# retir/Style-Big-GAN

Hardware: AMD Instinct MI355X
Metric: images/sec (G+D step) StyleGAN2-ADA 256x256 bf16 (higher is better)
Workload: dtype bf16; 1 GPU; configs/sg2ada.yaml @ 256x256: sg2_classic G (skip) + D (orig), softplus + R1(0.01)/4, idle Greg slot /16 (G lr x 16/17), global batch 64 = 1 rank(s) x 2 round(s) x batch_gpu 32 (the rounds of a phase evaluated in one pass, minibatch-std groups and loss those of the separate rounds), bf16 from 8x8 up (num_fp16_res 6; the reference recipe defaults to 4), conv_clamp 256, ADA off; global_batch=64, per_rank_batch=64, parallelism=dp1

## Files before the change

### include/sbg_hip.h

```cpp
#ifndef SBG_HIP_H
#define SBG_HIP_H

#include <stdint.h>

#ifdef __cplusplus
extern "C" {
#endif

typedef void* sbg_stream_t;

enum sbg_status {
    SBG_OK = 0,
    SBG_ERR_INVALID = 1,
    SBG_ERR_UNSUPPORTED = 2,
    SBG_ERR_LAUNCH = 3
};

enum sbg_dtype { SBG_F32 = 0, SBG_F16 = 1, SBG_BF16 = 2 };

enum sbg_act {
    SBG_ACT_LINEAR = 1, SBG_ACT_RELU = 2, SBG_ACT_LRELU = 3, SBG_ACT_TANH = 4, SBG_ACT_SIGMOID = 5,
    SBG_ACT_ELU = 6, SBG_ACT_SELU = 7, SBG_ACT_SOFTPLUS = 8, SBG_ACT_SWISH = 9
};

// ... 14 lines not shown
    float gain;
    int     inSize[4];      int64_t inStride[4];
    int     filterSize[2];  int     filterStride[2];
    int     outSize[4];     int64_t outStride[4];
    const float* oscale; const float* noise; int64_t noise_stride_n; const float* bias;
    int act; float alpha, act_gain, clamp;
    int     filter_exact16;
    const void* dact_y; float* dact_partial; int dact_act; float dact_alpha, dact_gain, dact_clamp;
    const float* post_scale;
} sbg_upfirdn2d_params;
int sbg_upfirdn2d_tail_supported(const sbg_upfirdn2d_params* p);
int64_t sbg_upfirdn2d_dact_rows(const sbg_upfirdn2d_params* p);
int sbg_upfirdn2d(const sbg_upfirdn2d_params* p, sbg_stream_t stream);

int sbg_upfirdn2d_separable_supported(int up, int down, int taps);
int sbg_upfirdn2d_separable(const float* x, const float* f, float* y, int M, int IH, int IW, int OH, int OW, int taps,
                            int up, int down, int padx0, int pady0, int flip, float gain, sbg_stream_t stream);

#define SBG_MAX_TAPS 16
typedef struct sbg_conv_params {
    const void* x; const void* w; void* y;
    const float* oscale;
    int xdtype, ydtype;
    int N, IH, IW, Cin, Cout, OH, OW;
    int64_t xs_n, xs_h, xs_w;
    int64_t ys_n, ys_h, ys_w;
    int64_t ws_slab, ws_co;
    int stride;
    int ntaps;
    int tap_dy[SBG_MAX_TAPS], tap_dx[SBG_MAX_TAPS], tap_slab[SBG_MAX_TAPS];
    int accumulate;
    const float* bias; const float* noise; int64_t noise_stride_n;
    int act; float alpha, gain, clamp;
    void* workspace; int ksplit;
    int nphase; int ph_ntaps[4], ph_oh[4], ph_ow[4]; int64_t ph_yoff[4];
} sbg_conv_params;
int64_t sbg_conv2d_igemm_workspace(const sbg_conv_params* p);
int     sbg_conv2d_igemm(const sbg_conv_params* p, sbg_stream_t stream);


typedef struct sbg_wgrad_params {
    const void* a; const void* b; float* out; void* workspace;
    int dtype;
    int N, PH, PW, Ca, BH, BW, Cb;
    int64_t as_n, as_h, as_w;
    int64_t bs_n, bs_h, bs_w;
    int stride;
    int ntaps;
    int tap_dy[SBG_MAX_TAPS], tap_dx[SBG_MAX_TAPS];
    int accumulate;
} sbg_wgrad_params;
int64_t sbg_conv2d_wgrad_workspace(const sbg_wgrad_params* p);
int     sbg_conv2d_wgrad(const sbg_wgrad_params* p, sbg_stream_t stream);


int sbg_scale_nc(const void* x, const float* a, const float* z, void* y, int dtype, int layout,
                 int N, int C, int64_t HW, int64_t z_stride_n, sbg_stream_t stream);
int sbg_scale_shift_nc(const void* x, const float* a, const float* b, void* y, int dtype, int layout,
                       int N, int C, int64_t HW, sbg_stream_t stream);

int sbg_dot_hw_splits(int layout, int N, int C, int64_t HW);
int sbg_dot_hw(const void* u, const void* v, float* partial, int dtype, int layout,
               int N, int C, int64_t HW, sbg_stream_t stream);
int sbg_moments_hw(const void* x, float* r, int dtype, int N, int C, int64_t HW, sbg_stream_t stream);

typedef struct sbg_gg_problem {
    const float *a0, *b0, *a1, *b1;
    float* c; const float* bias; float* rowsum;
    int64_t a0_rs, a0_cs, b0_rs, b0_cs, a1_rs, a1_cs, b1_rs, b1_cs, c_rs, c_cs;
    int M, N, K0, K1, nterms;
    float alpha0, alpha1, bias_scale, rowsum_scale;
} sbg_gg_problem;
int sbg_grouped_gemm(const sbg_gg_problem* problems, int count, sbg_stream_t stream);

int sbg_dot_hw_scale_supported(int C);
int sbg_dot_hw_scale(const void* u, const void* v, const float* scale, void* y, float* partial, int dtype,
                     int N, int C, int64_t HW, sbg_stream_t stream);


int sbg_modconv_bwd_supported(int C);
int sbg_modconv_bwd(const void* dy, const void* y, const float* dcoef, const float* noise, const float* bias,
                    void* d2, float* partial, float* dnoise, int dtype, int N, int C, int64_t HW, int64_t noise_stride_n,
                    int act, float alpha, float gain, float clamp, sbg_stream_t stream);
int sbg_modconv_bwd_prescaled(const void* dy, const void* y, const float* prescale, const float* dcoef, const float* noise, const float* bias,
                              void* d2, float* partial, float* partial3, float* dnoise, int dtype, int N, int C, int64_t HW,
                              int64_t noise_stride_n, int act, float alpha, float gain, float clamp, sbg_stream_t stream);

int64_t sbg_sn_workspace(int rows, int cols);
int sbg_sn_power_iteration(const float* W, const float* u, float* v, float* u_new, float* sigma, void* workspace,
                           int rows, int cols, float eps, sbg_stream_t stream);

int64_t sbg_mbstd_workspace(int N, int C, int HW, int G, int F);
int sbg_mbstd_fwd(const float* x, float* y, void* workspace, int N, int C, int HW, int G, int F, sbg_stream_t stream);
int sbg_mbstd_bwd(const float* x, const float* dy, float* dx, int N, int C, int HW, int G, int F, sbg_stream_t stream);

int sbg_split_bf16_cat(const float* x, void* y, int64_t outer, int64_t C, int64_t inner, int nseg, const int* order, sbg_stream_t stream);
int sbg_split_bf16_cat_nd(const float* x, const int64_t* shape, const int64_t* xstrides, int cat_dim, void* y, int nseg, const int* order, sbg_stream_t stream);

int sbg_attention_supported(int Q, int M, int D, int DV);
int sbg_attention_fwd(const float* theta, const float* phi, const float* g, float* out, int N, int Q, int M, int D, int DV,
                      sbg_stream_t stream);
int sbg_attention_bwd_supported(int Q, int M, int D, int DV);
int64_t sbg_attention_bwd_workspace(int N, int Q);
int sbg_attention_bwd(const float* theta, const float* phi, const float* g, const float* dout, float* dtheta, float* dphi, float* dg,
                      void* workspace, int N, int Q, int M, int D, int DV, sbg_stream_t stream);

// ... 152 lines not shown
```

### style-big-gan_amd/_lib.py

```python
import ctypes
import os
import threading

import torch

_HERE = os.path.dirname(os.path.abspath(__file__))
LIB_PATH = os.environ.get("SBG_HIP_LIBRARY") or os.path.join(_HERE, "libsbg_hip.so")

SBG_F32, SBG_F16, SBG_BF16 = 0, 1, 2
SBG_MAX_TAPS = 16

_DTYPES = {torch.float32: SBG_F32, torch.float16: SBG_F16, torch.bfloat16: SBG_BF16}


def dtype_code(dtype):
    try:
        return _DTYPES[dtype]
    except KeyError:
        raise RuntimeError(f"style_big_gan_amd: unsupported dtype {dtype} (float32 / float16 / bfloat16 only)")


class UpfirdnParams(ctypes.Structure):
    _fields_ = [
        ("x", ctypes.c_void_p), ("f", ctypes.c_void_p), ("y", ctypes.c_void_p),
# ... 60 lines not shown
class GgProblem(ctypes.Structure):
    _fields_ = [("a0", ctypes.c_void_p), ("b0", ctypes.c_void_p), ("a1", ctypes.c_void_p), ("b1", ctypes.c_void_p),
                ("c", ctypes.c_void_p), ("bias", ctypes.c_void_p), ("rowsum", ctypes.c_void_p),
                ("a0_rs", ctypes.c_int64), ("a0_cs", ctypes.c_int64), ("b0_rs", ctypes.c_int64), ("b0_cs", ctypes.c_int64),
                ("a1_rs", ctypes.c_int64), ("a1_cs", ctypes.c_int64), ("b1_rs", ctypes.c_int64), ("b1_cs", ctypes.c_int64),
                ("c_rs", ctypes.c_int64), ("c_cs", ctypes.c_int64),
                ("M", ctypes.c_int), ("N", ctypes.c_int), ("K0", ctypes.c_int), ("K1", ctypes.c_int), ("nterms", ctypes.c_int),
                ("alpha0", ctypes.c_float), ("alpha1", ctypes.c_float), ("bias_scale", ctypes.c_float), ("rowsum_scale", ctypes.c_float)]


class ProfRecord(ctypes.Structure):
    _fields_ = [("kind", ctypes.c_int), ("dims", ctypes.c_int * 7), ("flops", ctypes.c_double), ("bytes", ctypes.c_double),
                ("ms", ctypes.c_float), ("pad", ctypes.c_int)]


KERNEL_KINDS = {1: "bias_act", 2: "upfirdn2d", 3: "conv_igemm", 4: "conv_wgrad", 5: "wgrad_reduce", 6: "scale_nc", 7: "dot_hw", 9: "sn_power", 10: "attention",
                11: "grid_sample", 12: "filter1d", 13: "color", 14: "weight_prep", 15: "torgb", 16: "fromrgb", 17: "grouped_gemm", 18: "ppl",
                19: "projector", 20: "image_export", 21: "resample", 22: "pr", 23: "grad_finish", 24: "resident", 25: "diffaug", 26: "nn_u8", 27: "swd", 28: "spectrum",
                29: "msssim"}
MSSSIM_VARIANTS = {0: "level", 1: "down", 2: "merge"}
SWD_VARIANTS = {0: "pyr_down", 1: "pyr_lap", 2: "gather", 3: "moments", 4: "project", 5: "l1", 6: "merge"}
SPECTRUM_VARIANTS = {0: "rows", 1: "cols"}
NN_VARIANTS = {0: "norms", 1: "single", 2: "split", 3: "merge"}
RESIDENT_PATHS = {1: "dword", 2: "byte"}
PPL_VARIANTS = {0: "slerp", 1: "lerp", 2: "prep", 3: "dist"}
PROJ_VARIANTS = {0: "reg", 1: "reg_bwd", 2: "normalize", 3: "sqdist", 4: "sqdist_bwd"}
IMG_VARIANTS = {0: "quantize_tile", 1: "truncate_mix"}
QUANT_RULES = {"grid": 0, "clamp": 1}
RESAMPLE_VARIANTS = {0: "h", 1: "v"}
PR_VARIANTS = {0: "single", 1: "split", 2: "merge", 3: "norms"}
GRAD_FINISH_VARIANTS = {0: "sweep", 1: "merge"}
DIFFAUG_VARIANTS = {0: "sum", 1: "apply", 2: "adj_sum", 3: "adj_apply", 4: "single", 5: "adj_single"}
DIFFAUG_WORDS = 12
ATT_VARIANTS = {0: "single", 1: "stream", 2: "stream_stats", 3: "stream_dq", 4: "stream_dkv"}

_lib = None
_lock = threading.Lock()

_c = ctypes
SYMBOLS = [
    ("sbg_version", _c.c_int, []),
    ("sbg_last_error", _c.c_char_p, []),
    ("sbg_bias_act", _c.c_int, [_c.c_void_p] * 6 + [_c.c_int, _c.c_int, _c.c_int, _c.c_float, _c.c_float, _c.c_float,
                                                   _c.c_int64, _c.c_int, _c.c_int64, _c.c_void_p]),
    ("sbg_upfirdn2d_tail_supported", _c.c_int, [_c.POINTER(UpfirdnParams)]),
    ("sbg_upfirdn2d", _c.c_int, [_c.POINTER(UpfirdnParams), _c.c_void_p]),
    ("sbg_upfirdn2d_dact_rows", _c.c_int64, [_c.POINTER(UpfirdnParams)]),
    ("sbg_upfirdn2d_separable_supported", _c.c_int, [_c.c_int] * 3),
    ("sbg_upfirdn2d_separable", _c.c_int, [_c.c_void_p] * 3 + [_c.c_int] * 11 + [_c.c_float, _c.c_void_p]),
    ("sbg_conv2d_igemm_workspace", _c.c_int64, [_c.POINTER(ConvParams)]),
    ("sbg_conv2d_igemm", _c.c_int, [_c.POINTER(ConvParams), _c.c_void_p]),
    ("sbg_conv2d_wgrad_workspace", _c.c_int64, [_c.POINTER(WgradParams)]),
    ("sbg_conv2d_wgrad", _c.c_int, [_c.POINTER(WgradParams), _c.c_void_p]),
    ("sbg_scale_nc", _c.c_int, [_c.c_void_p] * 4 + [_c.c_int, _c.c_int, _c.c_int, _c.c_int, _c.c_int64, _c.c_int64, _c.c_void_p]),
    ("sbg_scale_shift_nc", _c.c_int, [_c.c_void_p] * 4 + [_c.c_int, _c.c_int, _c.c_int, _c.c_int, _c.c_int64, _c.c_void_p]),
    ("sbg_sn_workspace", _c.c_int64, [_c.c_int, _c.c_int]),
    ("sbg_sn_power_iteration", _c.c_int, [_c.c_void_p] * 6 + [_c.c_int, _c.c_int, _c.c_float, _c.c_void_p]),
    ("sbg_mbstd_workspace", _c.c_int64, [_c.c_int] * 5),
    ("sbg_mbstd_fwd", _c.c_int, [_c.c_void_p] * 3 + [_c.c_int] * 5 + [_c.c_void_p]),
    ("sbg_mbstd_bwd", _c.c_int, [_c.c_void_p] * 3 + [_c.c_int] * 5 + [_c.c_void_p]),
    ("sbg_split_bf16_cat", _c.c_int, [_c.c_void_p, _c.c_void_p, _c.c_int64, _c.c_int64, _c.c_int64, _c.c_int, _c.POINTER(_c.c_int), _c.c_void_p]),
    ("sbg_split_bf16_cat_nd", _c.c_int, [_c.c_void_p, _c.POINTER(_c.c_int64), _c.POINTER(_c.c_int64), _c.c_int, _c.c_void_p, _c.c_int, _c.POINTER(_c.c_int), _c.c_void_p]),
    ("sbg_attention_supported", _c.c_int, [_c.c_int] * 4),
    ("sbg_attention_fwd", _c.c_int, [_c.c_void_p] * 4 + [_c.c_int] * 5 + [_c.c_void_p]),
    ("sbg_attention_bwd_supported", _c.c_int, [_c.c_int] * 4),
    ("sbg_attention_bwd_workspace", _c.c_int64, [_c.c_int, _c.c_int]),
    ("sbg_attention_bwd", _c.c_int, [_c.c_void_p] * 8 + [_c.c_int] * 5 + [_c.c_void_p]),
    ("sbg_dot_hw_splits", _c.c_int, [_c.c_int, _c.c_int, _c.c_int, _c.c_int64]),
    ("sbg_dot_hw", _c.c_int, [_c.c_void_p] * 3 + [_c.c_int, _c.c_int, _c.c_int, _c.c_int, _c.c_int64, _c.c_void_p]),
    ("sbg_moments_hw", _c.c_int, [_c.c_void_p, _c.c_void_p, _c.c_int, _c.c_int, _c.c_int, _c.c_int64, _c.c_void_p]),
    ("sbg_grouped_gemm", _c.c_int, [_c.c_void_p, _c.c_int, _c.c_void_p]),
    ("sbg_dot_hw_scale_supported", _c.c_int, [_c.c_int]),
    ("sbg_dot_hw_scale", _c.c_int, [_c.c_void_p] * 5 + [_c.c_int, _c.c_int, _c.c_int, _c.c_int64, _c.c_void_p]),
    ("sbg_modconv_bwd_supported", _c.c_int, [_c.c_int]),
    ("sbg_modconv_bwd", _c.c_int, [_c.c_void_p] * 8 + [_c.c_int, _c.c_int, _c.c_int, _c.c_int64, _c.c_int64, _c.c_int, _c.c_float, _c.c_float, _c.c_float, _c.c_void_p]),
    ("sbg_modconv_bwd_prescaled", _c.c_int, [_c.c_void_p] * 10 + [_c.c_int, _c.c_int, _c.c_int, _c.c_int64, _c.c_int64, _c.c_int, _c.c_float, _c.c_float, _c.c_float, _c.c_void_p]),
    ("sbg_pack_weight", _c.c_int, [_c.c_void_p, _c.c_void_p, _c.c_int, _c.c_int, _c.c_int, _c.c_int, _c.c_int] + [_c.c_int64] * 4
     + [_c.c_int, _c.c_float, _c.c_void_p, _c.c_void_p]),
    ("sbg_unpack_wgrad", _c.c_int, [_c.c_void_p, _c.c_int64, _c.c_int64, _c.c_void_p, _c.c_void_p, _c.c_void_p] + [_c.c_int] * 4
     + [_c.c_int64] * 4 + [_c.c_float, _c.c_void_p]),
    ("sbg_demod_coefs", _c.c_int, [_c.c_void_p] * 3 + [_c.c_int] * 3 + [_c.c_float, _c.c_void_p]),
    ("sbg_demod_coefs_bwd", _c.c_int, [_c.c_void_p] * 6 + [_c.c_int] * 3 + [_c.c_void_p]),
    ("sbg_torgb_supported", _c.c_int, [_c.c_int, _c.c_int]),
    ("sbg_torgb_bwd_blocks", _c.c_int, [_c.c_int, _c.c_int, _c.c_int64]),
    ("sbg_torgb_fwd", _c.c_int, [_c.c_void_p] * 4 + [_c.c_int] * 4 + [_c.c_int64, _c.c_float, _c.c_void_p]),
    ("sbg_torgb_bwd", _c.c_int, [_c.c_void_p] * 6 + [_c.c_int] * 4 + [_c.c_int64, _c.c_float, _c.c_void_p]),
    ("sbg_fromrgb_supported", _c.c_int, [_c.c_int] * 3),
    ("sbg_fromrgb_bwd_blocks", _c.c_int, [_c.c_int, _c.c_int64]),
    ("sbg_fromrgb_fwd", _c.c_int, [_c.c_void_p] * 4 + [_c.c_int] * 4 + [_c.c_int64, _c.c_int, _c.c_float, _c.c_float, _c.c_float, _c.c_void_p]),
    ("sbg_fromrgb_bwd", _c.c_int, [_c.c_void_p] * 6 + [_c.c_int] * 4 + [_c.c_int64, _c.c_int, _c.c_float, _c.c_float, _c.c_float, _c.c_void_p]),
    ("sbg_grid_sample2d", _c.c_int, [_c.POINTER(GridSampleParams), _c.c_void_p]),
    ("sbg_grid_sample2d_bwd", _c.c_int, [_c.POINTER(GridSampleParams), _c.c_void_p]),
    ("sbg_grid_sample2d_bwd_overwrites", _c.c_int, [_c.POINTER(GridSampleParams)]),
    ("sbg_color_transform", _c.c_int, [_c.c_void_p] * 3 + [_c.c_int, _c.c_int64, _c.c_void_p]),
    ("sbg_filter1d_batch", _c.c_int, [_c.c_void_p] * 3 + [_c.c_int] * 8 + [_c.c_void_p]),
    ("sbg_ppl_slerp_endpoints", _c.c_int, [_c.c_void_p] * 3 + [_c.c_float, _c.c_void_p, _c.c_int, _c.c_int, _c.c_void_p]),
    ("sbg_ppl_lerp_endpoints", _c.c_int, [_c.c_void_p] * 3 + [_c.c_float, _c.c_void_p, _c.c_int, _c.c_int64, _c.c_void_p]),
    ("sbg_ppl_prep_images", _c.c_int, [_c.c_void_p] * 2 + [_c.c_int] * 4 + [_c.c_int64] * 4 + [_c.c_int, _c.c_int, _c.c_void_p]),
    ("sbg_ppl_dist_workspace", _c.c_int64, [_c.c_int, _c.c_int64]),
    ("sbg_ppl_dist", _c.c_int, [_c.c_void_p] * 3 + [_c.c_int, _c.c_int64, _c.c_float, _c.c_void_p]),
    ("sbg_proj_noise_reg_workspace", _c.c_int64, [_c.c_void_p, _c.c_int]),
    ("sbg_proj_noise_reg", _c.c_int, [_c.c_void_p] * 2 + [_c.c_int] + [_c.c_void_p] * 4),
    ("sbg_proj_noise_reg_bwd", _c.c_int, [_c.c_void_p] * 3 + [_c.c_int] + [_c.c_void_p] * 4),
    ("sbg_proj_noise_normalize_workspace", _c.c_int64, [_c.c_void_p, _c.c_int]),
    ("sbg_proj_noise_normalize", _c.c_int, [_c.c_void_p] * 2 + [_c.c_int] + [_c.c_void_p] * 2),
    ("sbg_proj_sqdist_workspace", _c.c_int64, [_c.c_int64]),
# ... 113 lines not shown
```

### style-big-gan_amd/csrc/conv_wgrad.hip

```cpp
#include "conv_common.h"
#include "lds_asm.h"

namespace {

using sbgconv::bf16_mfma; using sbgconv::f16_mfma; using sbgconv::Mfma;

struct WgradArgs {
    const unsigned short* a; const unsigned short* b; float* out; float* ws;
    int N, PH, PW, Ca, BH, BW, Cb;
    int64_t as_n, as_h, as_w, bs_n, bs_h, bs_w;
    int stride, ntaps;
    int tap_dy[SBG_MAX_TAPS], tap_dx[SBG_MAX_TAPS];
    int accumulate;
    int64_t P;
    int nchunks;
    int nsplit, chunks_per_split;
    int atiles, btiles;
    int tap0;
    int ntaps_total;
};

static __device__ __forceinline__ bool wgrad_decode_block(const WgradArgs& p, int& ta, int& tb, int& split)
{
    const int T = p.atiles * p.btiles;
// ... 102 lines not shown
    };

    if (chunk_begin < chunk_end) {
        issue_loads(chunk_begin);
        for (int c = chunk_begin; c < chunk_end; c++) {
            write_tiles();
            __syncthreads();
            if (c + 1 < chunk_end) issue_loads(c + 1);
            short8_t fa[TA];
#pragma unroll
            for (int i = 0; i < TA; i++) fa[i] = read_frag(sA, RSA, wa + 16 * i);
#pragma unroll
            for (int t = 0; t < NT; t++) {
                if (t < p.ntaps) {
                    short8_t fb[TB];
#pragma unroll
                    for (int j = 0; j < TB; j++) fb[j] = read_frag(sB + t * B_BYTES, RSB, wb + 16 * j);
#pragma unroll
                    for (int i = 0; i < TA; i++)
#pragma unroll
                        for (int j = 0; j < TB; j++) acc[t][i][j] = Mfma<MF>::run(fa[i], fb[j], acc[t][i][j]);
                }
            }
            __syncthreads();
        }
    }

    const bool direct = (p.nsplit == 1);
    float* dst_base = direct ? p.out : p.ws + (int64_t)split * p.ntaps_total * p.Ca * p.Cb;
#pragma unroll
    for (int t = 0; t < NT; t++) {
        if (t >= p.ntaps) continue;
        float* slab = dst_base + (int64_t)(p.tap0 + t) * p.Ca * p.Cb;
#pragma unroll
        for (int i = 0; i < TA; i++)
#pragma unroll
            for (int j = 0; j < TB; j++) {
                const int cb = cb0 + wb + 16 * j + fi;
                if (cb >= p.Cb) continue;
#pragma unroll
                for (int e = 0; e < 4; e++) {
                    const int ca = ca0 + wa + 16 * i + 4 * fg + e;
                    if (ca >= p.Ca) continue;
                    float* d = slab + (int64_t)ca * p.Cb + cb;
                    const float v = acc[t][i][j][e];
                    *d = (direct && p.accumulate) ? *d + v : v;
                }
            }
    }
}



using sbgconv::lds_void_ptr;

template <class MF, int S, int BCA, int NSTAGE>
__global__ __launch_bounds__(512) void conv_wgrad_rows_kernel(WgradArgs p, unsigned a_bytes, unsigned b_bytes)
{
    static_assert(BCA == 64 || BCA == 128, "a tile of 64 or 128 channels");
    static_assert(NSTAGE >= 2 && NSTAGE <= 6, "2..6 stages (the wait ladder covers five chunks in flight)");
    constexpr int BCB = 64, NT = 9, DEPTH = NSTAGE - 1;
    constexpr int TA = BCA / 32;
    constexpr int APIECES = BCA / 16;
    constexpr int PCOLS = S * 31 + 3;
    constexpr int PPR = (PCOLS + 7) / 8;
    constexpr int PROW = PPR * 8;
    constexpr int NWAVE = 8;
    constexpr int NPIECE = ((APIECES + 3 * PPR + NWAVE - 1) / NWAVE) * NWAVE;
    constexpr int PIECES = NPIECE / NWAVE;
    constexpr int NREAL = APIECES + 3 * PPR;
    constexpr int A_BYTES = APIECES * 1024, STAGE = NREAL * 1024, DUMP = NSTAGE * STAGE;

    extern __shared__ __attribute__((aligned(16))) unsigned char smem[];
    const int tid = threadIdx.x, lane = tid & 63;
    const int wave = __builtin_amdgcn_readfirstlane(tid >> 6);
    int ta_, tb_, split;
    if (!wgrad_decode_block(p, ta_, tb_, split)) return;
    const int ca0 = ta_ * BCA, cb0 = tb_ * BCB;
    const int chunk_begin = split * p.chunks_per_split;
    int chunk_end = chunk_begin + p.chunks_per_split;
    if (chunk_end > p.nchunks) chunk_end = p.nchunks;
    const int nloc = chunk_end - chunk_begin;
    const int xblocks = p.PW >> 5;
    const int dy0 = p.tap_dy[0], dx0 = p.tap_dx[0];

    __amdgpu_buffer_rsrc_t ar = __builtin_amdgcn_make_buffer_rsrc((void*)p.a, 0, (int)a_bytes, 0x00020000);
    __amdgpu_buffer_rsrc_t br = __builtin_amdgcn_make_buffer_rsrc((void*)p.b, 0, (int)b_bytes, 0x00020000);

    const int drow = lane >> 3, dchunk = lane & 7;
    auto src_chunk = [&](int R) { return (((dchunk >> 1) ^ ((R >> 1) & 3)) << 1) | (dchunk & 1); };

    struct ChunkC { int py, n, px0; unsigned char* st; };
    auto chunk_coords = [&](int loc) -> ChunkC {
        const int c = chunk_begin + loc;
        const int xb = c % xblocks, rowid = c / xblocks;
        ChunkC r; r.py = rowid % p.PH; r.n = rowid / p.PH; r.px0 = xb << 5; r.st = smem + (loc % NSTAGE) * STAGE;
        return r;
    };
    auto issue_piece = [&](const ChunkC& cc, int i) {
        const int py = cc.py, n = cc.n, px0 = cc.px0;
        unsigned char* st = cc.st;
        {
            const int piece = wave + NWAVE * i;
            if (piece < APIECES) {
                const int R = (piece & 3) * 8 + drow;
                const int ch = ca0 + (piece >> 2) * 64 + src_chunk(R) * 8;
                const unsigned okm = 0u - (unsigned)(ch < p.Ca);
                const unsigned real = (unsigned)(n * (int)p.as_n + py * (int)p.as_h + (px0 + R) * (int)p.as_w + ch) * 2u;
                __builtin_amdgcn_raw_ptr_buffer_load_lds(ar, (lds_void_ptr)(st + piece * 1024), 16, (real & okm) | (SBG_OOB_OFFSET & ~okm), 0, 0, 0);
            } else {
                const int q = piece - APIECES;
                const int r = q / PPR, jb = q - r * PPR;
                const int R = r * PROW + jb * 8 + drow;
                constexpr int NEVEN = (PCOLS + 1) / 2, EVROWS = ((NEVEN + 7) / 8) * 8;
                const int pcol = (S == 1) ? jb * 8 + drow : (jb * 8 < EVROWS ? 2 * (jb * 8 + drow) : 2 * (jb * 8 - EVROWS + drow) + 1);
                const int by = S * py + dy0 + r, bx = S * px0 + dx0 + pcol;
                const int ch = cb0 + src_chunk(R) * 8;
                const unsigned okm = 0u - (unsigned)((q < 3 * PPR) & (pcol < PCOLS) & ((unsigned)by < (unsigned)p.BH) & ((unsigned)bx < (unsigned)p.BW) & (ch < p.Cb));
                const unsigned real = (unsigned)(n * (int)p.bs_n + by * (int)p.bs_h + bx * (int)p.bs_w + ch) * 2u;
                unsigned char* dst = (q < 3 * PPR) ? st + A_BYTES + q * 1024 : smem + DUMP;
                __builtin_amdgcn_raw_ptr_buffer_load_lds(br, (lds_void_ptr)dst, 16, (real & okm) | (SBG_OOB_OFFSET & ~okm), 0, 0, 0);
            }
        }
    };
    auto issue = [&](int loc) {
        const ChunkC cc = chunk_coords(loc);
#pragma unroll
        for (int i = 0; i < PIECES; i++) issue_piece(cc, i);
    };
    constexpr bool late = true;

    const int wa = (wave >> 2) * (BCA / 2), wb = (wave & 3) * 16;
    const int fi = lane & 15, fg = lane >> 4, fq = fi >> 2, fp = fi & 3;
    const unsigned lds_base = (unsigned)(uintptr_t)((lds_void_ptr)smem);
    float4_t acc[NT][TA];
#pragma unroll
    for (int t = 0; t < NT; t++)
#pragma unroll
        for (int i = 0; i < TA; i++) acc[t][i] = float4_t{0.f, 0.f, 0.f, 0.f};

    auto frag_off = [&](int Rrel, int col) {
        const int chunk = (col >> 3) + (fp >> 1);
        const int sw = (((chunk >> 1) ^ ((Rrel >> 1) & 3)) << 1) | (chunk & 1);
        return Rrel * 128 + sw * 16 + (fp & 1) * 8;
    };
    int offA[TA], offB[3];
#pragma unroll
    for (int i = 0; i < TA; i++) {
        const int col = wa + 16 * i;
        offA[i] = (col >> 6) * 4096 + frag_off(4 * fg + fq, col & 63);
    }
#pragma unroll
    for (int d = 0; d < 3; d++) {
        constexpr int EVROWS_ = (((PCOLS + 1) / 2 + 7) / 8) * 8;
        offB[d] = frag_off((S == 1 ? d : (d & 1) * EVROWS_ + (d >> 1)) + 4 * fg + fq, wb);
    }
    auto read_frag = [&](const unsigned char* base, int off, int hi_off) -> short8_t {
        short4_t lo = lds_tr_read(base + off), hi = lds_tr_read(base + off + hi_off);
        return short8_t{lo[0], lo[1], lo[2], lo[3], hi[0], hi[1], hi[2], hi[3]};
    };

#pragma unroll
    for (int s = 0; s < DEPTH; s++) if (s < nloc) issue(s);
    for (int s = 0; s < nloc; s++) {
        {
            const int later = nloc - 1 - s;
            if (DEPTH >= 2 && later >= DEPTH - 1) asm volatile("s_waitcnt vmcnt(%0)" :: "n"((DEPTH - 1) * PIECES) : "memory");
            else if (DEPTH >= 3 && later == DEPTH - 2) asm volatile("s_waitcnt vmcnt(%0)" :: "n"((DEPTH >= 3 ? DEPTH - 2 : 0) * PIECES) : "memory");
            else if (DEPTH >= 4 && later == DEPTH - 3) asm volatile("s_waitcnt vmcnt(%0)" :: "n"((DEPTH >= 4 ? DEPTH - 3 : 0) * PIECES) : "memory");
            else if (DEPTH >= 5 && later == DEPTH - 4) asm volatile("s_waitcnt vmcnt(%0)" :: "n"((DEPTH >= 5 ? DEPTH - 4 : 0) * PIECES) : "memory");
            else                                       asm volatile("s_waitcnt vmcnt(0)" ::: "memory");
        }
        __builtin_amdgcn_s_barrier();
        const bool more = s + DEPTH < nloc;
        ChunkC nxt = chunk_coords(more ? s + DEPTH : s);
        if (more && !late) {
#pragma unroll
            for (int i = 0; i < PIECES; i++) issue_piece(nxt, i);
        }
        const unsigned stage = lds_base + (unsigned)((s % NSTAGE) * STAGE);
        short4_t alo[TA], ahi[TA], blo[3], bhi[3];
        sbg_static_for<TA>([&](auto it) {
            constexpr int i = decltype(it)::value;
            lds_tr_issue<0>(alo[i], stage + (unsigned)offA[i]);
            lds_tr_issue<16 * 128>(ahi[i], stage + (unsigned)offA[i]);
        });
        unsigned pb[3];
#pragma unroll
        for (int d = 0; d < 3; d++) pb[d] = stage + (unsigned)offB[d];
        auto issue_b = [&](auto tt) {
            constexpr int t = decltype(tt)::value, dyi = t / 3, dxi = t % 3, OFF = A_BYTES + dyi * PROW * 128;
            lds_tr_issue<OFF>(blo[t % 3], pb[dxi]);
            lds_tr_issue<OFF + 16 * 128>(bhi[t % 3], pb[dxi]);
        };
        issue_b(std::integral_constant<int, 0>{});
        issue_b(std::integral_constant<int, 1>{});
        sbg_static_for<9>([&](auto tt) {
            constexpr int t = decltype(tt)::value;
            if constexpr (t + 2 < 9) issue_b(std::integral_constant<int, t + 2>{});
            lds_wait<(t + 2 < 9 ? 4 : t + 1 < 9 ? 2 : 0)>(blo[t % 3], bhi[t % 3]);
            const short8_t fb = short8_t{blo[t % 3][0], blo[t % 3][1], blo[t % 3][2], blo[t % 3][3], bhi[t % 3][0], bhi[t % 3][1], bhi[t % 3][2], bhi[t % 3][3]};
#pragma unroll
            for (int i = 0; i < TA; i++) {
                const short8_t fa_i = short8_t{alo[i][0], alo[i][1], alo[i][2], alo[i][3], ahi[i][0], ahi[i][1], ahi[i][2], ahi[i][3]};
                acc[t][i] = Mfma<MF>::run(fa_i, fb, acc[t][i]);
            }
            if (more && late) {
                sbg_static_for<PIECES>([&](auto pt) {
                    constexpr int i = decltype(pt)::value;
                    if constexpr (i * 9 / PIECES == t) issue_piece(nxt, i);
                });
            }
        });
    }

    const bool direct = (p.nsplit == 1);
    float* dst_base = direct ? p.out : p.ws + (int64_t)split * p.ntaps_total * p.Ca * p.Cb;
    const int cb = cb0 + wb + fi;
#pragma unroll
    for (int t = 0; t < NT; t++) {
        if (t >= p.ntaps || cb >= p.Cb) continue;
        float* slab = dst_base + (int64_t)(p.tap0 + t) * p.Ca * p.Cb;
#pragma unroll
        for (int i = 0; i < TA; i++)
#pragma unroll
            for (int e = 0; e < 4; e++) {
                const int ca = ca0 + wa + 16 * i + 4 * fg + e;
                if (ca >= p.Ca) continue;
                float* d = slab + (int64_t)ca * p.Cb + cb;
                const float v = acc[t][i][e];
                *d = (direct && p.accumulate) ? *d + v : v;
            }
    }
}

template <int LANES>
__global__ __launch_bounds__(256) void wgrad_reduce_kernel(const float* ws, float* out, int64_t n, int nsplit, int accumulate)
{
    const int sub = threadIdx.x % LANES;
    const int64_t step = (int64_t)gridDim.x * (256 / LANES);
    for (int64_t i = (int64_t)blockIdx.x * (256 / LANES) + threadIdx.x / LANES; i < n; i += step) {
        float s = 0.f;
        int k = sub;
        for (; k + 7 * LANES < nsplit; k += 8 * LANES) {
            float v[8];
#pragma unroll
// ... 52 lines not shown
                v = *reinterpret_cast<const short8_t*>(p.b + (int64_t)n * p.bs_n + (int64_t)by * p.bs_h + (int64_t)bx * p.bs_w + ch);
            *reinterpret_cast<short8_t*>(lb + piece * 8) = v;
        }
        __builtin_amdgcn_s_waitcnt(0xC07F);
        __builtin_amdgcn_wave_barrier();
        short8_t fa[TA];
#pragma unroll
        for (int i = 0; i < TA; i++)
#pragma unroll
            for (int j = 0; j < 8; j++) fa[i][j] = (short)la[(8 * fg + j) * p.Ca + 16 * i + fi];
#pragma unroll
        for (int t = 0; t < 9; t++) {
            if (t < p.ntaps) {
                const unsigned short* row = lb + (tdy[t] * PCOLS + tdx[t]) * p.Cb;
#pragma unroll
                for (int jb = 0; jb < TB; jb++) {
                    short8_t fb;
#pragma unroll
                    for (int j = 0; j < 8; j++) fb[j] = (short)row[(p.stride * (8 * fg + j)) * p.Cb + 16 * jb + fi];
#pragma unroll
                    for (int i = 0; i < TA; i++) acc[t][i][jb] = Mfma<MF>::run(fa[i], fb, acc[t][i][jb]);
                }
            }
        }
        __builtin_amdgcn_wave_barrier();
    }
    float* dst = p.ws + (int64_t)slab * p.ntaps_total * p.Ca * p.Cb;
#pragma unroll
    for (int t = 0; t < 9; t++) {
        if (t < p.ntaps) {
#pragma unroll
            for (int i = 0; i < TA; i++)
#pragma unroll
                for (int jb = 0; jb < TB; jb++)
#pragma unroll
                    for (int e = 0; e < 4; e++) {
                        const int ca = 16 * i + 4 * fg + e, cb = 16 * jb + fi;
                        if (ca < p.Ca && cb < p.Cb) dst[((int64_t)(p.tap0 + t) * p.Ca + ca) * p.Cb + cb] = acc[t][i][jb][e];
                    }
        }
    }
}


enum WgradFamily { WG_EMPTY, WG_THIN, WG_ROWS, WG_BIG, WG_TAPS };

struct WgradPlan {
    WgradFamily family;
    int bca, bcb;
    int atiles, btiles, nchunks, nsplit, chunks_per_split;
    int64_t grid; int block, lds;
    int code;
    unsigned a_bytes, b_bytes;
    int dymin, dxmin, RY, PCOLS, wave_lds;
    double flops_per_tap, bytes_ab, bytes_out_per_tap;
};

static bool thin_plan(const sbg_wgrad_params& q, WgradPlan& pl)
{
    if (q.Ca > 32 || q.Cb > 32 || q.Ca * q.Cb > 512 || q.ntaps > 9 || q.stride > 2) return false;
    int dy0 = q.tap_dy[0], dy1 = dy0, dx0 = q.tap_dx[0], dx1 = dx0;
    for (int i = 1; i < q.ntaps; i++) {
        if (q.tap_dy[i] < dy0) dy0 = q.tap_dy[i]; if (q.tap_dy[i] > dy1) dy1 = q.tap_dy[i];
        if (q.tap_dx[i] < dx0) dx0 = q.tap_dx[i]; if (q.tap_dx[i] > dx1) dx1 = q.tap_dx[i];
    }
    const int64_t nchunks = (int64_t)q.N * q.PH * ((q.PW + 31) / 32);
    if (dy1 - dy0 > 2 || dx1 - dx0 > 2 || nchunks >= INT32_MAX) return false;
    pl.dymin = dy0; pl.dxmin = dx0; pl.RY = dy1 - dy0 + 1; pl.PCOLS = q.stride * 31 + (dx1 - dx0) + 1;
    pl.wave_lds = ((32 * q.Ca + pl.RY * pl.PCOLS * q.Cb) * 2 + 15) & ~15;
    pl.grid = (nchunks + 15) / 16;
    if (pl.grid > 2048) pl.grid = 2048;
    return true;
}

static bool rows_kernel_ok(const sbg_wgrad_params& q, WgradPlan& pl)
{
    if (q.stride > 2 || (q.PW % 32) != 0 || q.ntaps != 9) return false;
    for (int t = 0; t < 9; t++)
        if (q.tap_dy[t] != q.tap_dy[0] + t / 3 || q.tap_dx[t] != q.tap_dx[0] + t % 3) return false;
    if (q.as_n < 0 || q.as_h < 0 || q.as_w < 0 || q.bs_n < 0 || q.bs_h < 0 || q.bs_w < 0) return false;
    auto extent = [&](int h, int w, int c, int64_t s_n, int64_t s_h, int64_t s_w) { return 2 * ((int64_t)(q.N - 1) * s_n + (int64_t)(h - 1) * s_h + (int64_t)(w - 1) * s_w + c); };
    const int64_t ab = extent(q.PH, q.PW, q.Ca, q.as_n, q.as_h, q.as_w), bb = extent(q.BH, q.BW, q.Cb, q.bs_n, q.bs_h, q.bs_w);
    pl.a_bytes = (unsigned)ab; pl.b_bytes = (unsigned)bb;
    return ab < (int64_t)SBG_OOB_OFFSET && bb < (int64_t)SBG_OOB_OFFSET;
}

static constexpr int rows_nstage(int stride, int bca)
{
    if (bca == 128) return 4;
    return stride == 1 ? 4 : 2;
}

static void plan_split(WgradPlan& pl, const sbg_wgrad_params& q, int bca, int bcb, int target)
{
    pl.bca = bca; pl.bcb = bcb;
    pl.atiles = (q.Ca + bca - 1) / bca;
    pl.btiles = (q.Cb + bcb - 1) / bcb;
    const int tiles = pl.atiles * pl.btiles;
    int want = (target + tiles - 1) / tiles;
    int maxsplit = pl.nchunks / 8; if (maxsplit < 1) maxsplit = 1;
    if (want > maxsplit) want = maxsplit;
    if (want < 1) want = 1;
    pl.chunks_per_split = (pl.nchunks + want - 1) / want;
    pl.nsplit = (pl.nchunks + pl.chunks_per_split - 1) / pl.chunks_per_split;
    pl.grid = 8 * (int64_t)tiles * ((pl.nsplit + 7) / 8);
}

static WgradPlan wgrad_plan(const sbg_wgrad_params& q)
{
    WgradPlan pl = {};
    const int64_t P = (int64_t)q.N * q.PH * q.PW;
    pl.family = WG_EMPTY; pl.nsplit = 1;
    if (P == 0) return pl;
    pl.nchunks = (int)((P + 31) / 32);
    pl.block = 256;
    if (thin_plan(q, pl)) {
        pl.family = WG_THIN;
        pl.bca = (q.Ca + 15) / 16; pl.bcb = (q.Cb + 15) / 16;
        pl.atiles = pl.btiles = 1; pl.nsplit = 4 * (int)pl.grid; pl.chunks_per_split = 0;
        pl.lds = 4 * pl.wave_lds;
        pl.code = 3000000 + pl.bca * 10 + pl.bcb;
    } else if (rows_kernel_ok(q, pl)) {
        pl.family = WG_ROWS;
        plan_split(pl, q, q.Ca >= 128 ? 128 : 64, 64, 512);
        const int stage_kib = pl.bca / 16 + 3 * ((q.stride * 31 + 3 + 7) / 8);
        pl.block = 512;
        pl.lds = (rows_nstage(q.stride, pl.bca) * stage_kib + 1) * 1024;
        pl.code = 1000000 + pl.bca * 1000 + 64;
    } else {
        pl.family = q.ntaps == 1 ? WG_BIG : WG_TAPS;
        const int tile = pl.family == WG_BIG ? 128 : 64, nt = pl.family == WG_BIG ? 1 : 9;
        plan_split(pl, q, tile, tile, 1024);
        pl.lds = (1 + nt) * 32 * (tile * 2 + 32);
        pl.code = tile * 1000 + tile;
    }
    pl.flops_per_tap = 2.0 * (double)P * q.Ca * (double)q.Cb;
    pl.bytes_ab = 2.0 * (double)P * q.Ca + 2.0 * (double)q.N * q.BH * q.BW * q.Cb;
    pl.bytes_out_per_tap = 4.0 * (double)q.Ca * q.Cb * (pl.nsplit > 1 ? pl.nsplit : 1);
    return pl;
}

static int fill_args(const sbg_wgrad_params* q, WgradPlan& pl, WgradArgs& a)
{
    SBG_CHECK(q && q->a && q->b && q->out, "conv2d_wgrad: null pointer");
    SBG_CHECK(q->dtype == SBG_BF16 || q->dtype == SBG_F16, "conv2d_wgrad: a/b must be bf16 or f16 (fp32 inputs are split by the host)");
    SBG_CHECK(q->N >= 0 && q->PH >= 1 && q->PW >= 1 && q->BH >= 1 && q->BW >= 1, "conv2d_wgrad: bad sizes");
    SBG_CHECK(q->Ca >= 8 && q->Cb >= 8 && (q->Ca % 8) == 0 && (q->Cb % 8) == 0, "conv2d_wgrad: channel counts must be multiples of 8 (pad on the host)");
    SBG_CHECK(q->ntaps >= 1 && q->ntaps <= SBG_MAX_TAPS, "conv2d_wgrad: 1..%d taps", SBG_MAX_TAPS);
    SBG_CHECK(q->stride >= 1, "conv2d_wgrad: stride must be >= 1");
    SBG_CHECK(sbg_aligned16(q->a) && sbg_aligned16(q->b), "conv2d_wgrad: a and b must be 16-byte aligned");
    SBG_CHECK((q->as_n % 8) == 0 && (q->as_h % 8) == 0 && (q->as_w % 8) == 0 && (q->bs_n % 8) == 0 && (q->bs_h % 8) == 0 && (q->bs_w % 8) == 0,
              "conv2d_wgrad: pixel / row strides must be multiples of 8 elements");
    pl = wgrad_plan(*q);
    a.a = (const unsigned short*)q->a; a.b = (const unsigned short*)q->b; a.out = q->out; a.ws = (float*)q->workspace;
    a.N = q->N; a.PH = q->PH; a.PW = q->PW; a.Ca = q->Ca; a.BH = q->BH; a.BW = q->BW; a.Cb = q->Cb;
    a.as_n = q->as_n; a.as_h = q->as_h; a.as_w = q->as_w; a.bs_n = q->bs_n; a.bs_h = q->bs_h; a.bs_w = q->bs_w;
    a.stride = q->stride; a.ntaps = q->ntaps; a.accumulate = q->accumulate;
    for (int t = 0; t < SBG_MAX_TAPS; t++) { a.tap_dy[t] = q->tap_dy[t]; a.tap_dx[t] = q->tap_dx[t]; }
    a.P = (int64_t)q->N * q->PH * q->PW;
    a.tap0 = 0; a.ntaps_total = q->ntaps;
    a.nchunks = pl.nchunks; a.nsplit = pl.nsplit; a.chunks_per_split = pl.chunks_per_split; a.atiles = pl.atiles; a.btiles = pl.btiles;
    return SBG_OK;
}

template <auto Kern, class... Extra>
static int launch(const WgradPlan& pl, const WgradArgs& g, hipStream_t s, const Extra&... extra)
{
    return sbgconv::launch_as<Kern>(SBG_K_CONV_WGRAD, "conv2d_wgrad", pl.grid, 1, pl.block, pl.lds, s,
                                    pl.flops_per_tap * g.ntaps, pl.bytes_ab + pl.bytes_out_per_tap * g.ntaps,
                                    {(int)(g.P > INT32_MAX ? INT32_MAX : g.P), g.Ca, g.Cb, g.ntaps, g.stride, g.nsplit, pl.code}, g, extra...);
}

template <class MF, int TA, int TB>
static int thin(const WgradPlan& pl, const WgradArgs& a, hipStream_t s) { return launch<conv_wgrad_thin_kernel<MF, TA, TB>>(pl, a, s, pl.dymin, pl.dxmin, pl.RY, pl.PCOLS, pl.wave_lds); }
template <class MF, int S, int BCA>
static int rows(const WgradPlan& pl, const WgradArgs& a, hipStream_t s) { return launch<conv_wgrad_rows_kernel<MF, S, BCA, rows_nstage(S, BCA)>>(pl, a, s, pl.a_bytes, pl.b_bytes); }

template <int LANES>
static int reduce_slabs(const WgradArgs& a, int64_t n, hipStream_t s)
{
    return sbgconv::launch_as<wgrad_reduce_kernel<LANES>>(SBG_K_WGRAD_REDUCE, "conv2d_wgrad", sbg_stream_grid(n * LANES, 256), 1, 256, 0, s, 0.0,
                                                          4.0 * n * (a.nsplit + 1), {(int)n, a.nsplit}, a.ws, a.out, n, a.nsplit, a.accumulate);
}
static int reduce_slabs(const WgradArgs& a, hipStream_t s)
{
    const int64_t n = (int64_t)a.ntaps_total * a.Ca * a.Cb;
    if (n >= (1 << 18) || a.nsplit < 16) return reduce_slabs<1>(a, n, s);
    return n >= (1 << 14) ? reduce_slabs<4>(a, n, s) : reduce_slabs<64>(a, n, s);
}

template <class MF>
static int run(const WgradPlan& pl, const WgradArgs& a, hipStream_t s)
{
    int rc = SBG_OK;
    if (pl.family == WG_THIN)
        rc = pl.bca == 1 ? (pl.bcb == 1 ? thin<MF, 1, 1>(pl, a, s) : thin<MF, 1, 2>(pl, a, s)) : (pl.bcb == 1 ? thin<MF, 2, 1>(pl, a, s) : thin<MF, 2, 2>(pl, a, s));
    else if (pl.family == WG_ROWS)
        rc = a.stride == 1 ? (pl.bca == 64 ? rows<MF, 1, 64>(pl, a, s) : rows<MF, 1, 128>(pl, a, s)) : (pl.bca == 64 ? rows<MF, 2, 64>(pl, a, s) : rows<MF, 2, 128>(pl, a, s));
    else if (pl.family == WG_BIG)
        rc = launch<conv_wgrad_kernel<MF, 128, 128, 1>>(pl, a, s);
    else
        for (int t0 = 0; t0 < a.ntaps && rc == SBG_OK; t0 += 9) {
            WgradArgs g = a;
            g.tap0 = t0; g.ntaps = (a.ntaps - t0 < 9) ? a.ntaps - t0 : 9;
            for (int t = 0; t < g.ntaps; t++) { g.tap_dy[t] = a.tap_dy[t0 + t]; g.tap_dx[t] = a.tap_dx[t0 + t]; }
            rc = launch<conv_wgrad_kernel<MF, 64, 64, 9>>(pl, g, s);
        }
    return rc != SBG_OK || pl.nsplit == 1 ? rc : reduce_slabs(a, s);
}

}

extern "C" int64_t sbg_conv2d_wgrad_workspace(const sbg_wgrad_params* q)
{
    WgradPlan pl; WgradArgs a;
    if (fill_args(q, pl, a) != SBG_OK) return -1;
    if (pl.nsplit <= 1) return 0;
    return (int64_t)pl.nsplit * q->ntaps * q->Ca * q->Cb * (int64_t)sizeof(float);
}

extern "C" int sbg_conv2d_wgrad(const sbg_wgrad_params* q, sbg_stream_t stream)
{
    WgradPlan pl; WgradArgs a;
    const int rc = fill_args(q, pl, a);
    if (rc != SBG_OK) return rc;
    hipStream_t s = (hipStream_t)stream;
    if (pl.family == WG_EMPTY) {
        if (!a.accumulate && hipMemsetAsync(a.out, 0, (size_t)a.ntaps_total * a.Ca * a.Cb * sizeof(float), s) != hipSuccess)
            return sbg_fail(SBG_ERR_LAUNCH, "conv2d_wgrad: memset failed");
        return SBG_OK;
    }
    SBG_CHECK(pl.nsplit == 1 || a.ws != nullptr, "conv2d_wgrad: workspace required (%d pixel splits)", pl.nsplit);
    return q->dtype == SBG_BF16 ? run<bf16_mfma>(pl, a, s) : run<f16_mfma>(pl, a, s);
}
```

Measured before the change: 634.7 img/s.

## Route 4-pixel-wide stride-1 weight gradients through the rows kernel

Extends the pipelined rows wgrad kernel with a narrow-image mode for stride-1 convolutions on 4-pixel-wide maps (the 4x4 layers). Each chunk now packs several image rows, spanning two images when needed, into a padded patch layout with its own pitch and swizzle. These layers previously fell back to the generic taps or thin kernels. The split count is planned against a larger target so the small problem still fills the GPU. It also adds a query entry point, which nothing in this change calls, and brings more template instantiations and fiddly index and bounds logic.

```diff
diff --git a/include/sbg_hip.h b/include/sbg_hip.h
--- a/include/sbg_hip.h
+++ b/include/sbg_hip.h
@@ -90,6 +90,7 @@
 } sbg_wgrad_params;
 int64_t sbg_conv2d_wgrad_workspace(const sbg_wgrad_params* p);
 int     sbg_conv2d_wgrad(const sbg_wgrad_params* p, sbg_stream_t stream);
+int     sbg_conv2d_wgrad_narrow(const sbg_wgrad_params* p);
 
 
 int sbg_scale_nc(const void* x, const float* a, const float* z, void* y, int dtype, int layout,
diff --git a/style-big-gan_amd/_lib.py b/style-big-gan_amd/_lib.py
--- a/style-big-gan_amd/_lib.py
+++ b/style-big-gan_amd/_lib.py
@@ -136,6 +136,7 @@
     ("sbg_conv2d_igemm", _c.c_int, [_c.POINTER(ConvParams), _c.c_void_p]),
     ("sbg_conv2d_wgrad_workspace", _c.c_int64, [_c.POINTER(WgradParams)]),
     ("sbg_conv2d_wgrad", _c.c_int, [_c.POINTER(WgradParams), _c.c_void_p]),
+    ("sbg_conv2d_wgrad_narrow", _c.c_int, [_c.POINTER(WgradParams)]),
     ("sbg_scale_nc", _c.c_int, [_c.c_void_p] * 4 + [_c.c_int, _c.c_int, _c.c_int, _c.c_int, _c.c_int64, _c.c_int64, _c.c_void_p]),
     ("sbg_scale_shift_nc", _c.c_int, [_c.c_void_p] * 4 + [_c.c_int, _c.c_int, _c.c_int, _c.c_int, _c.c_int64, _c.c_void_p]),
     ("sbg_sn_workspace", _c.c_int64, [_c.c_int, _c.c_int]),
diff --git a/style-big-gan_amd/csrc/conv_wgrad.hip b/style-big-gan_amd/csrc/conv_wgrad.hip
--- a/style-big-gan_amd/csrc/conv_wgrad.hip
+++ b/style-big-gan_amd/csrc/conv_wgrad.hip
@@ -178,9 +178,10 @@
 
 
 
+
 using sbgconv::lds_void_ptr;
 
-template <class MF, int S, int BCA, int NSTAGE>
+template <class MF, int S, int BCA, int NSTAGE, int NW = 0>
 __global__ __launch_bounds__(512) void conv_wgrad_rows_kernel(WgradArgs p, unsigned a_bytes, unsigned b_bytes)
 {
     static_assert(BCA == 64 || BCA == 128, "a tile of 64 or 128 channels");
@@ -192,9 +193,16 @@
     constexpr int PPR = (PCOLS + 7) / 8;
     constexpr int PROW = PPR * 8;
     constexpr int NWAVE = 8;
-    constexpr int NPIECE = ((APIECES + 3 * PPR + NWAVE - 1) / NWAVE) * NWAVE;
+    static_assert(NW == 0 || (S == 1 && NW == 4), "narrow images: stride 1, 4 pixels wide");
+    constexpr int NWD = NW ? NW : 32;
+    constexpr int LGNW = NW == 16 ? 4 : NW == 8 ? 3 : 2, RPS = NW == 16 ? 2 : 4, NSEG = NW ? 32 / (NWD * RPS) : 1;
+    constexpr int PITCH = NW ? ((NW + 2 + 7) / 8) * 8 : PROW, SEGROWS = (RPS + 2) * PITCH;
+    constexpr int HI_ROWS = NW ? (16 / NWD / RPS) * SEGROWS + (16 / NWD % RPS) * PITCH : 16;
+    static_assert(PITCH % 8 == 0 && HI_ROWS % 8 == 0 && (NW == 0 || NSEG * SEGROWS == 96), "swizzle term per tap column; 96 patch rows");
+    constexpr int PATCHP = NW ? NSEG * SEGROWS / 8 : 3 * PPR;
+    constexpr int NPIECE = ((APIECES + PATCHP + NWAVE - 1) / NWAVE) * NWAVE;
     constexpr int PIECES = NPIECE / NWAVE;
-    constexpr int NREAL = APIECES + 3 * PPR;
+    constexpr int NREAL = APIECES + PATCHP;
     constexpr int A_BYTES = APIECES * 1024, STAGE = NREAL * 1024, DUMP = NSTAGE * STAGE;
 
     extern __shared__ __attribute__((aligned(16))) unsigned char smem[];
@@ -216,17 +224,47 @@
     const int drow = lane >> 3, dchunk = lane & 7;
     auto src_chunk = [&](int R) { return (((dchunk >> 1) ^ ((R >> 1) & 3)) << 1) | (dchunk & 1); };
 
-    struct ChunkC { int py, n, px0; unsigned char* st; };
+    struct ChunkC { int py, n, px0; unsigned char* st; int py1, n1; };
     auto chunk_coords = [&](int loc) -> ChunkC {
         const int c = chunk_begin + loc;
-        const int xb = c % xblocks, rowid = c / xblocks;
-        ChunkC r; r.py = rowid % p.PH; r.n = rowid / p.PH; r.px0 = xb << 5; r.st = smem + (loc % NSTAGE) * STAGE;
-        return r;
+        if constexpr (NW != 0) {
+            const int row0 = c * (32 / NWD);
+            ChunkC r; r.n = row0 / p.PH; r.py = row0 - r.n * p.PH; r.px0 = 0; r.st = smem + (loc % NSTAGE) * STAGE;
+            const bool next = r.py + RPS >= p.PH;
+            r.n1 = next ? r.n + 1 : r.n; r.py1 = next ? 0 : r.py + RPS;
+            return r;
+        } else {
+            const int xb = c % xblocks, rowid = c / xblocks;
+            ChunkC r; r.py = rowid % p.PH; r.n = rowid / p.PH; r.px0 = xb << 5; r.st = smem + (loc % NSTAGE) * STAGE; r.py1 = r.n1 = 0;
+            return r;
+        }
     };
     auto issue_piece = [&](const ChunkC& cc, int i) {
         const int py = cc.py, n = cc.n, px0 = cc.px0;
         unsigned char* st = cc.st;
-        {
+        if constexpr (NW != 0) {
+            const int piece = wave + NWAVE * i;
+            if (piece < APIECES) {
+                const int R = (piece & 3) * 8 + drow;
+                const int rl = R >> LGNW, seg = rl / RPS;
+                const int sn = seg ? cc.n1 : n, sy = (seg ? cc.py1 : py) + rl % RPS;
+                const int ch = ca0 + (piece >> 2) * 64 + src_chunk(R) * 8;
+                const unsigned okm = 0u - (unsigned)((sn < p.N) & (ch < p.Ca));
+                const unsigned real = (unsigned)(sn * (int)p.as_n + sy * (int)p.as_h + (R & (NW - 1)) * (int)p.as_w + ch) * 2u;
+                __builtin_amdgcn_raw_ptr_buffer_load_lds(ar, (lds_void_ptr)(st + piece * 1024), 16, (real & okm) | (SBG_OOB_OFFSET & ~okm), 0, 0, 0);
+            } else {
+                const int q = piece - APIECES;
+                const int R = q * 8 + drow;
+                const int seg = R / SEGROWS, rem = R - seg * SEGROWS, prow = rem / PITCH, pcol = rem - prow * PITCH;
+                const int sn = seg ? cc.n1 : n;
+                const int by = (seg ? cc.py1 : py) + dy0 + prow, bx = dx0 + pcol;
+                const int ch = cb0 + src_chunk(R) * 8;
+                const unsigned okm = 0u - (unsigned)((q < PATCHP) & (pcol < NW + 2) & (sn < p.N) & ((unsigned)by < (unsigned)p.BH) & ((unsigned)bx < (unsigned)p.BW) & (ch < p.Cb));
+                const unsigned real = (unsigned)(sn * (int)p.bs_n + by * (int)p.bs_h + bx * (int)p.bs_w + ch) * 2u;
+                unsigned char* dst = (q < PATCHP) ? st + A_BYTES + q * 1024 : smem + DUMP;
+                __builtin_amdgcn_raw_ptr_buffer_load_lds(br, (lds_void_ptr)dst, 16, (real & okm) | (SBG_OOB_OFFSET & ~okm), 0, 0, 0);
+            }
+        } else {
             const int piece = wave + NWAVE * i;
             if (piece < APIECES) {
                 const int R = (piece & 3) * 8 + drow;
@@ -279,7 +317,9 @@
 #pragma unroll
     for (int d = 0; d < 3; d++) {
         constexpr int EVROWS_ = (((PCOLS + 1) / 2 + 7) / 8) * 8;
-        offB[d] = frag_off((S == 1 ? d : (d & 1) * EVROWS_ + (d >> 1)) + 4 * fg + fq, wb);
+        const int pix = 4 * fg + fq;
+        if constexpr (NW != 0) offB[d] = frag_off((pix >> LGNW) * PITCH + (pix & (NW - 1)) + d, wb);
+        else offB[d] = frag_off((S == 1 ? d : (d & 1) * EVROWS_ + (d >> 1)) + 4 * fg + fq, wb);
     }
     auto read_frag = [&](const unsigned char* base, int off, int hi_off) -> short8_t {
         short4_t lo = lds_tr_read(base + off), hi = lds_tr_read(base + off + hi_off);
@@ -315,9 +355,9 @@
 #pragma unroll
         for (int d = 0; d < 3; d++) pb[d] = stage + (unsigned)offB[d];
         auto issue_b = [&](auto tt) {
-            constexpr int t = decltype(tt)::value, dyi = t / 3, dxi = t % 3, OFF = A_BYTES + dyi * PROW * 128;
+            constexpr int t = decltype(tt)::value, dyi = t / 3, dxi = t % 3, OFF = A_BYTES + dyi * PITCH * 128;
             lds_tr_issue<OFF>(blo[t % 3], pb[dxi]);
-            lds_tr_issue<OFF + 16 * 128>(bhi[t % 3], pb[dxi]);
+            lds_tr_issue<OFF + HI_ROWS * 128>(bhi[t % 3], pb[dxi]);
         };
         issue_b(std::integral_constant<int, 0>{});
         issue_b(std::integral_constant<int, 1>{});
@@ -476,6 +516,7 @@
     int64_t grid; int block, lds;
     int code;
     unsigned a_bytes, b_bytes;
+    int narrow;
     int dymin, dxmin, RY, PCOLS, wave_lds;
     double flops_per_tap, bytes_ab, bytes_out_per_tap;
 };
@@ -497,9 +538,15 @@
     return true;
 }
 
+static int rows_narrow_width(const sbg_wgrad_params& q)
+{
+    return q.stride == 1 && q.PW == 4 && q.PH % 4 == 0 ? 4 : 0;
+}
+
 static bool rows_kernel_ok(const sbg_wgrad_params& q, WgradPlan& pl)
 {
-    if (q.stride > 2 || (q.PW % 32) != 0 || q.ntaps != 9) return false;
+    pl.narrow = rows_narrow_width(q);
+    if (q.stride > 2 || ((q.PW % 32) != 0 && !pl.narrow) || q.ntaps != 9) return false;
     for (int t = 0; t < 9; t++)
         if (q.tap_dy[t] != q.tap_dy[0] + t / 3 || q.tap_dx[t] != q.tap_dx[0] + t % 3) return false;
     if (q.as_n < 0 || q.as_h < 0 || q.as_w < 0 || q.bs_n < 0 || q.bs_h < 0 || q.bs_w < 0) return false;
@@ -515,13 +562,14 @@
     return stride == 1 ? 4 : 2;
 }
 
-static void plan_split(WgradPlan& pl, const sbg_wgrad_params& q, int bca, int bcb, int target)
+static void plan_split(WgradPlan& pl, const sbg_wgrad_params& q, int bca, int bcb, int target, int count_bca = 0)
 {
     pl.bca = bca; pl.bcb = bcb;
     pl.atiles = (q.Ca + bca - 1) / bca;
     pl.btiles = (q.Cb + bcb - 1) / bcb;
     const int tiles = pl.atiles * pl.btiles;
-    int want = (target + tiles - 1) / tiles;
+    const int counted = count_bca ? ((q.Ca + count_bca - 1) / count_bca) * pl.btiles : tiles;
+    int want = (target + counted - 1) / counted;
     int maxsplit = pl.nchunks / 8; if (maxsplit < 1) maxsplit = 1;
     if (want > maxsplit) want = maxsplit;
     if (want < 1) want = 1;
@@ -546,12 +594,14 @@
         pl.code = 3000000 + pl.bca * 10 + pl.bcb;
     } else if (rows_kernel_ok(q, pl)) {
         pl.family = WG_ROWS;
-        plan_split(pl, q, q.Ca >= 128 ? 128 : 64, 64, 512);
-        const int stage_kib = pl.bca / 16 + 3 * ((q.stride * 31 + 3 + 7) / 8);
+        if (pl.narrow) plan_split(pl, q, q.Ca >= 128 ? 128 : 64, 64, 1024, 64);
+        else plan_split(pl, q, q.Ca >= 128 ? 128 : 64, 64, 512);
+        const int stage_kib = pl.bca / 16 + (pl.narrow ? 12 : 3 * ((q.stride * 31 + 3 + 7) / 8));
         pl.block = 512;
         pl.lds = (rows_nstage(q.stride, pl.bca) * stage_kib + 1) * 1024;
         pl.code = 1000000 + pl.bca * 1000 + 64;
     } else {
+        pl.narrow = 0;
         pl.family = q.ntaps == 1 ? WG_BIG : WG_TAPS;
         const int tile = pl.family == WG_BIG ? 128 : 64, nt = pl.family == WG_BIG ? 1 : 9;
         plan_split(pl, q, tile, tile, 1024);
@@ -597,8 +647,13 @@
 
 template <class MF, int TA, int TB>
 static int thin(const WgradPlan& pl, const WgradArgs& a, hipStream_t s) { return launch<conv_wgrad_thin_kernel<MF, TA, TB>>(pl, a, s, pl.dymin, pl.dxmin, pl.RY, pl.PCOLS, pl.wave_lds); }
-template <class MF, int S, int BCA>
-static int rows(const WgradPlan& pl, const WgradArgs& a, hipStream_t s) { return launch<conv_wgrad_rows_kernel<MF, S, BCA, rows_nstage(S, BCA)>>(pl, a, s, pl.a_bytes, pl.b_bytes); }
+template <class MF, int S, int BCA, int NW = 0>
+static int rows(const WgradPlan& pl, const WgradArgs& a, hipStream_t s) { return launch<conv_wgrad_rows_kernel<MF, S, BCA, rows_nstage(S, BCA), NW>>(pl, a, s, pl.a_bytes, pl.b_bytes); }
+template <class MF, int BCA>
+static int rows_narrow(const WgradPlan& pl, const WgradArgs& a, hipStream_t s)
+{
+    return rows<MF, 1, BCA, 4>(pl, a, s);
+}
 
 template <int LANES>
 static int reduce_slabs(const WgradArgs& a, int64_t n, hipStream_t s)
@@ -619,6 +674,8 @@
     int rc = SBG_OK;
     if (pl.family == WG_THIN)
         rc = pl.bca == 1 ? (pl.bcb == 1 ? thin<MF, 1, 1>(pl, a, s) : thin<MF, 1, 2>(pl, a, s)) : (pl.bcb == 1 ? thin<MF, 2, 1>(pl, a, s) : thin<MF, 2, 2>(pl, a, s));
+    else if (pl.family == WG_ROWS && pl.narrow)
+        rc = pl.bca == 64 ? rows_narrow<MF, 64>(pl, a, s) : rows_narrow<MF, 128>(pl, a, s);
     else if (pl.family == WG_ROWS)
         rc = a.stride == 1 ? (pl.bca == 64 ? rows<MF, 1, 64>(pl, a, s) : rows<MF, 1, 128>(pl, a, s)) : (pl.bca == 64 ? rows<MF, 2, 64>(pl, a, s) : rows<MF, 2, 128>(pl, a, s));
     else if (pl.family == WG_BIG)
@@ -643,6 +700,12 @@
     return (int64_t)pl.nsplit * q->ntaps * q->Ca * q->Cb * (int64_t)sizeof(float);
 }
 
+extern "C" int sbg_conv2d_wgrad_narrow(const sbg_wgrad_params* q)
+{
+    WgradPlan pl; WgradArgs a;
+    return fill_args(q, pl, a) == SBG_OK && pl.family == WG_ROWS && pl.narrow != 0;
+}
+
 extern "C" int sbg_conv2d_wgrad(const sbg_wgrad_params* q, sbg_stream_t stream)
 {
     WgradPlan pl; WgradArgs a;
```

Measured after the change: 638.1 img/s, median of 6. About the same (+0.5%).
